# SashaYerashoff/evo-ssearch

Measured on NVIDIA B200. Metric: flat-IP top-k queries/sec @10M x 512 k=48, higher is better.
Workload: dtype f32

## Files before the change

evo-ssearch_b200/csrc/evs_api.cu:

```cuda
#include <errno.h>
#include <float.h>
#include <stdarg.h>
#include <stdio.h>
#include <stdlib.h>
#include <string.h>
#include <fcntl.h>
#include <sys/stat.h>
#include <unistd.h>

#include <atomic>
#include <mutex>
#include <new>
#include <string>
#include <thread>
#include <utility>
#include <vector>

#include "evs_internal.h"

using namespace evs;

static thread_local char t_err[512] = "";

static int fail(int code, const char* fmt, ...) {
// ... 1015 lines not shown
            const int rc2 = barrier_scan_done(idx->device, st);
            if (!rc) rc = rc2;
        }
        return rc;
    }
    const int kp = kp_override ? kp_override : pi.kp;
    const bool bf16 = idx->storage == EVS_STORE_BF16_F32;
    const bool shadow = pi.shadow && kp_override == 0;
    const bool scan_bf16 = bf16 && !shadow && kp_override == 0;
    const void* scan_rows = shadow ? (const void*)idx->xi8 : scan_bf16 ? idx->xb16 : (const void*)idx->xb32;
    const int qpp = shadow ? 1 : max_queries_per_pass(idx->d, scan_bf16);
    ScanPlan plan;
    CU(plan_scan(idx->ntotal, idx->d, shadow ? SCAN_I8 : scan_bf16, kp, qpp, idx->sm_count, tune, &plan));
    const int64_t chunk_cap = nq < kQueryChunk ? nq : kQueryChunk;
    int rc = ensure_dev(reinterpret_cast<unsigned long long**>(&idx->lists), &idx->lists_cap, (size_t)chunk_cap * plan.grid * kp);
    if (rc) return rc;
    if (kp_override == 0) {
        if ((rc = ensure_dev(&idx->margins_dev, &idx->margins_cap, (size_t)nq))) return rc;
        idx->last_nq = nq;
    }
    const bool fused = (kp_override ? (tune.fuse_finalize && nq == 1 && plan.variant == 1) : pi.fused) && !scan_only;
    if (out.x && out.x->merge_D && !fused) return fail(EVS_ECUDA, "internal: the exchange expected a fused single-query search");
    const float err_coef = (scan_bf16 || shadow) ? 0.f : gemv_err_coef(idx->d);
    if (shadow && !(fused && tune.pool_select && kp == 64))
        return fail(EVS_ECUDA, "internal: the int8 scan copy is searched by the fused pool kernel only");

    for (int64_t c0 = 0; c0 < nq; c0 += kQueryChunk) {
        const int64_t cn = (nq - c0) < kQueryChunk ? (nq - c0) : kQueryChunk;
        const float* qc = q_dev + (size_t)c0 * idx->d;
        ProfileScope prof;
        if ((rc = prof.begin(idx, profile, st))) return rc;
        FinalizeParams f = make_finalize(idx, idx->lists, plan.grid, kp, qc, k, out, c0, nq, err_coef);
        if (shadow) {
            f.shadow_emax = reinterpret_cast<const float*>(idx->words + W_EMAX);
            f.wide = idx->words + W_WIDE;
        }
        for (int64_t p0 = 0; p0 < cn; p0 += qpp) {
            ScanArgs a;
            a.xb = scan_rows;
            a.xs = shadow ? idx->xs8 : nullptr;
            a.is_bf16 = scan_bf16;
            a.is_i8 = shadow;
            a.n = idx->ntotal;
            a.d = idx->d;
            a.xq = qc;
            a.q0 = (int)p0;
            a.nq_pass = (int)((cn - p0) < qpp ? (cn - p0) : qpp);
            a.lists = idx->lists;
            a.kp = kp;
            if (fused) {
                a.fuse = &f;
                a.ticket = idx->words + W_TICKET;
                if (tune.pool_select && kp == 64) {
                    const size_t need = scan_pool_words(plan) + (shadow ? (size_t)idx->ntotal : 0);
                    if (idx->pool_cap < need) {
                        if (idx->pool) CU(cudaFree(idx->pool));
                        idx->pool = nullptr;
                        idx->pool_cap = 0;
                        CU(cudaMalloc(reinterpret_cast<void**>(&idx->pool), need * 8));
                        CU(cudaMemsetAsync(idx->pool, 0, need * 8, st));
                        idx->pool_cap = need;
                    }
                    a.pool = idx->pool;
                    if (small_shard_applies(idx, tune, kp, plan)) {
                        a.small_fast_cap = tune.small_fast_cap > 0 ? tune.small_fast_cap : 1;
                        if (out.q_host != nullptr) {
                            a.q_inline = out.q_host;
                            f.done_flag = out.done_flag;
                            f.done_seq = out.done_seq;
                        }
                    }
                }
                if (out.q_host != nullptr && a.q_inline == nullptr)
                    return fail(EVS_ECUDA, "internal: the host search expected the small-shard kernel");
                if (tune.scan_dynamic > 1 || (tune.scan_dynamic == 1 && a.pool != nullptr)) {
                    a.next_chunk = idx->words + W_NEXT_CHUNK;
                    a.chunk_groups = tune.scan_chunk_groups > 0 ? tune.scan_chunk_groups : 2;
                }
                if (tune.scan_clock) {
                    if ((rc = ensure_dev(&idx->cta_clock, &idx->cta_clock_cap, (size_t)plan.grid * 2 + 16))) return rc;
                    idx->cta_clock_n = plan.grid;
                    a.cta_clock = idx->cta_clock;
                    f.dbg = idx->cta_clock + (size_t)plan.grid * 2 + 8;
                }
            }
            CU(launch_scan(a, &plan, st));
        }
        if ((rc = prof.end(st))) return rc;
        if (scan_only || fused) continue;
        CU(launch_finalize(f, cn, st));
    }
    return EVS_OK;
}

__global__ void fill_final_kernel(float* D, long long* I, long long count) {
    for (long long i = (long long)blockIdx.x * blockDim.x + threadIdx.x; i < count; i += (long long)gridDim.x * blockDim.x) {
        D[i] = -FLT_MAX;
        I[i] = -1;
    }
}
__global__ void fill_partial_kernel(double* S, long long* I, long long count) {
    for (long long i = (long long)blockIdx.x * blockDim.x + threadIdx.x; i < count; i += (long long)gridDim.x * blockDim.x) {
        S[i] = -DBL_MAX;
        I[i] = -1;
    }
}

// ... 984 lines not shown
```

evo-ssearch_b200/csrc/evs_finalize.cuh:

```cuda
#pragma once
#include <float.h>

#include <type_traits>

#include "evs_common.cuh"
#include "evs_internal.h"

namespace evs {

__device__ __forceinline__ void st_release_sys_u64(unsigned long long* p, unsigned long long v) {
    asm volatile("st.release.sys.global.u64 [%0], %1;" ::"l"(p), "l"(v) : "memory");
}
__device__ __forceinline__ unsigned long long ld_acquire_sys_u64(const unsigned long long* p) {
    unsigned long long v;
    asm volatile("ld.acquire.sys.global.u64 %0, [%1];" : "=l"(v) : "l"(p) : "memory");
    return v;
}

__device__ __forceinline__ u64 score_rank_key(double s) { return f64_to_ordered(s == 0.0 ? 0.0 : s); }
__device__ __forceinline__ int better_i(u64 oa, long long ia, u64 ob, long long ib) {
    return (int)(oa > ob) | ((int)(oa == ob) & (int)(ia < ib));
}
__device__ __forceinline__ double widen_f32(float f) {
    const uint32_t u = __float_as_uint(f);
// ... 165 lines not shown
            }
            __nanosleep(20);
        }
        const double sv = __longlong_as_double((long long)(((unsigned long long)a.z << 32) | a.x));
        const long long iv = (long long)(((unsigned long long)b.z << 32) | b.x);
        sc[e] = sv;
        id[e] = iv;
        ok[e] = iv >= 0 ? score_rank_key(sv) : 0ull;
    }
    __syncthreads();
    if (*fail) {
        for (int r = threadIdx.x; r < k; r += blockDim.x) {
            D[(size_t)qi * k + r] = -FLT_MAX;
            I[(size_t)qi * k + r] = -1;
        }
        if (threadIdx.x == 0 && x.status) {
            *reinterpret_cast<volatile int*>(x.status) = *fail;
            __threadfence_system();
        }
        return;
    }
    for (int e = threadIdx.x; e < m; e += blockDim.x) {
        if (id[e] < 0) continue;
        atomicAdd(nvalid, 1);
        const int part = e / k;
        const long long it = id[e];
        const u64 ot = ok[e];
        int rank = e - part * k;
        for (int pp = 0; pp < x.world; pp++) {
            if (pp == part) continue;
            const int base = pp * k;
            int lo = 0, hi = k;
            while (lo < hi) {
                const int mid = (lo + hi) >> 1;
                const bool beats = id[base + mid] >= 0 && better_i(ok[base + mid], id[base + mid], ot, it);
                if (beats) lo = mid + 1;
                else hi = mid;
            }
            rank += lo;
        }
        if (rank < k) {
            D[(size_t)qi * k + rank] = (float)sc[e];
            I[(size_t)qi * k + rank] = it;
        }
    }
    __syncthreads();
    for (int r = *nvalid + threadIdx.x; r < k; r += blockDim.x) {
        D[(size_t)qi * k + r] = -FLT_MAX;
        I[(size_t)qi * k + r] = -1;
    }
}

template <int MAXR = 4, int UW = 0>
__device__ __forceinline__ void finalize_rank_emit(const FinalizeParams& p, long long qi, const u64* A, FinalizeShared* sh, double* sc,
                                                   long long* id, u64* ok, const double* qs, unsigned char* scratch, int kp_use = 0,
                                                   float shadow_E = 0.f, u64 cut = 0ull) {
    const int t = threadIdx.x, nt = blockDim.x;
    const int warp = t >> 5, lane = t & 31, nwarps = nt >> 5;
    const int kp = kp_use > 0 ? kp_use : p.kp;
    const float* xb32 = reinterpret_cast<const float*>(p.xb);
    const bool fastw = p.special != nullptr && __ldg(p.special) == 0u;
    auto rescore = [&](auto rtag, auto ftag) {
        constexpr int R = decltype(rtag)::value;
        constexpr bool FAST = decltype(ftag)::value;
        for (int c = R * warp; c < kp; c += R * nwarps) {
            u64 key[R];
            long long row[R];
            const float* xr[R];
            double sv[R];
#pragma unroll
            for (int r = 0; r < R; r++) {
                key[r] = (c + r < kp) ? A[c + r] : 0ull;
                row[r] = key[r] ? (long long)key_row(key[r]) : -1;
                xr[r] = (key[r] && !p.xb_is_bf16) ? xb32 + (size_t)row[r] * p.d : nullptr;
            }
            canon32_dot_multi<R, FAST, UW>(xr, qs, p.d, lane, sv);
            if (p.xb_is_bf16) {
                const __nv_bfloat16* xb16 = reinterpret_cast<const __nv_bfloat16*>(p.xb);
#pragma unroll
                for (int r = 0; r < R; r++) sv[r] = key[r] ? canon32_dot_bf16(xb16 + (size_t)row[r] * p.d, qs, p.d, lane) : -DBL_MAX;
            }
            if (lane == 0) {
#pragma unroll
                for (int r = 0; r < R; r++)
                    if (c + r < kp) {
                        sc[c + r] = sv[r];
                        id[c + r] = row[r];
                        ok[c + r] = row[r] >= 0 ? score_rank_key(sv[r]) : 0ull;
                    }
            }
        }
    };
    if (MAXR < 4 || 2 * nwarps >= kp) {
        if (fastw) rescore(std::integral_constant<int, 2>{}, std::true_type{});
        else rescore(std::integral_constant<int, 2>{}, std::false_type{});
    } else {
        if (fastw) rescore(std::integral_constant<int, MAXR < 4 ? 2 : 4>{}, std::true_type{});
        else rescore(std::integral_constant<int, MAXR < 4 ? 2 : 4>{}, std::false_type{});
    }
    __syncthreads();
    fin_stamp(p, 3);
    const bool want_margin = p.margins != nullptr || p.guard_count != nullptr || p.pred_slot != nullptr;
    for (int c = t; c < kp; c += nt)
        if (id[c] >= 0 && want_margin) atomicMax(&sh->maxerr, score_to_ordered((float)(sc[c] - widen_f32(key_score(A[c])))));
    __syncthreads();

    for (int c = t; c < kp; c += nt) {
        if (id[c] < 0) continue;
        atomicAdd(&sh->nvalid, 1);
        const double st = sc[c];
        const long long it = id[c];
        const u64 ot = ok[c];
        int rank = 0;
        for (int j = 0; j < kp; j++) rank += better_i(ok[j], id[j], ot, it) & (int)(id[j] >= 0);
        if (rank < p.k) {
            if (p.D) {
                p.D[(size_t)qi * p.k + rank] = (float)st;
                p.I[(size_t)qi * p.k + rank] = it + p.id_base;
            } else if (p.x.world > 0) {
                exchange_store_entry(p.x, (size_t)(p.x.q_off + qi) * p.k + rank, st, it + p.id_base, exchange_flag(p.x.seq));
            } else {
                p.P_scores[(size_t)qi * p.k + rank] = st;
                p.P_ids[(size_t)qi * p.k + rank] = it + p.id_base;
            }
            if (rank == p.k - 1 && want_margin && shadow_E > 0.f) {
                if (p.margins) p.margins[qi] = cut > 1ull ? (float)(st - widen_f32(key_score(cut))) - shadow_E : INFINITY;
            } else if (rank == p.k - 1 && want_margin) {
                const float worst = key_score(A[kp - 1]);
                const float under = fmaxf(ordered_to_score(sh->maxerr), 0.f);
                const float gap = (A[kp - 1] != 0ull) ? (float)(st - widen_f32(worst)) : INFINITY;
                const float margin = gap - under;
                if (p.margins) p.margins[qi] = margin;
                if (p.err_coef > 0.f) {
                    const float mx = p.max_norm ? *p.max_norm : 1.f;
                    const float B = sqrtf((float)sh->qnorm2) * 1.000001f * mx;
                    const bool certified = p.err_trunc > 0.f ? gap > p.err_trunc * (B + fabsf(worst)) + p.err_coef * B
                                                             : margin > p.err_coef * B;
                    if (!certified) sh->uncert = 1;
                }
            }
        }
    }
    __syncthreads();
    const int nvalid = sh->nvalid;
    for (int r = nvalid + t; r < p.k; r += nt) {
        if (p.D) {
            p.D[(size_t)qi * p.k + r] = -FLT_MAX;
            p.I[(size_t)qi * p.k + r] = -1;
        } else if (p.x.world > 0) {
            exchange_store_entry(p.x, (size_t)(p.x.q_off + qi) * p.k + r, -DBL_MAX, -1, exchange_flag(p.x.seq));
        } else {
            p.P_scores[(size_t)qi * p.k + r] = -DBL_MAX;
            p.P_ids[(size_t)qi * p.k + r] = -1;
        }
    }
    if (t == 0 && p.margins && nvalid < p.k) p.margins[qi] = INFINITY;
    if (t == 0) {
        const bool over = p.overflow != nullptr && p.overflow[qi] != 0;
        if (sh->uncert || over) {
            if (p.guard_count) {
                const int slot = atomicAdd(p.guard_count, 1);
                if (slot < p.guard_cap) {
                    p.guard_slot[qi] = slot;
                    p.guard_q[slot] = (int)qi;
                } else {
                    p.guard_slot[qi] = -2;
                    if (p.guard_cap > 0 && p.uncertified) atomicAdd(p.uncertified, 1ull);
                }
            } else if (p.uncertified) {
                atomicAdd(p.uncertified, 1ull);
            }
        }
    }
    fin_stamp(p, 4);
    if (p.x.world > 0 && p.D == nullptr) {
        if (t == 0) sh->nvalid = 0;
        if (p.x.merge_D != nullptr) {
            __syncthreads();
            exchange_merge(p.x, p.x.q_off + qi, p.x.nq_total, p.k, p.x.merge_D, p.x.merge_I, scratch,
                           &sh->fail, &sh->nvalid);
        }
    }
}



__device__ __forceinline__ void finalize_query(const FinalizeParams& p, long long qi, const u64* __restrict__ lists,
                                               unsigned char* smem_raw) {
    const int t = threadIdx.x, nt = blockDim.x;
    const int warp = t >> 5, lane = t & 31, nwarps = nt >> 5;
    const int kp = p.kp, L = p.L;
    const int scap = finalize_surv_cap(L, kp);
    FinalizeShared* sh = reinterpret_cast<FinalizeShared*>(smem_raw);
    u64* surv = reinterpret_cast<u64*>(smem_raw + sizeof(FinalizeShared));
    u64* pre = surv + finalize_surv_slots(L, kp);
    int* deep = reinterpret_cast<int*>(pre + 2 * (size_t)L);
    double* sc = reinterpret_cast<double*>(pre + 2 * (size_t)L + finalize_deep_slots(L));
    long long* id = reinterpret_cast<long long*>(sc + kp);
    u64* ok = reinterpret_cast<u64*>(id + kp);
    double* qs = reinterpret_cast<double*>(ok + kp);

    for (int l = t; l < L; l += nt) {
        const ulonglong2 v = __ldcg(reinterpret_cast<const ulonglong2*>(lists + (size_t)l * kp));
        pre[2 * l] = v.x;
        pre[2 * l + 1] = v.y;
    }
    if (qi == 0 && t == 0 && p.guard_count_next) *p.guard_count_next = 0;
    __syncthreads();
    fin_stamp(p, 0);
    if (p.err_coef > 0.f && warp == 0) {
        double s2 = 0.0;
        for (int i = lane; i < p.d; i += 32) s2 = fma(qs[i], qs[i], s2);
#pragma unroll
        for (int off = 16; off >= 1; off >>= 1) s2 += __shfl_xor_sync(0xffffffffu, s2, off);
        if (lane == 0) sh->qnorm2 = s2;
    }
    int hs = 1;
    while ((L / (hs * 2)) * 10 >= kp * 23) hs <<= 1;
    for (int attempt = 0; attempt < 2; attempt++) {
        if (attempt == 1) {
            if (sh->nsurv <= scap || hs == 1) break;
            __syncthreads();
            if (t == 0) {
                sh->nsurv = 0;
                sh->ndeep = 0;
                sh->T0 = 0ull;
            }
            hs = 1;
            __syncthreads();
        }
        const int Ls = (L + hs - 1) / hs;
        if (Ls >= kp) {
            int nper = 1;
            while (nper < 32 && nper * 2 * Ls <= nt) nper <<= 1;
            const int part = t & (nper - 1);
            for (int l0 = 0; l0 < Ls; l0 += nt / nper) {
                const int l = l0 + t / nper;
// ... 93 lines not shown
```

evo-ssearch_b200/csrc/evs_scan.cuh:

```cuda
#pragma once
#include "evs_common.cuh"
#include "evs_finalize.cuh"

namespace evs {

struct ScanParams {
    const void* xb;
    const float* xs;
    long long n;
    int d;
    const float* xq;
    int q0;
    u64* lists;
    int lists_stride_q;
    int kp;
    int tile_rows;
    int stages;
    unsigned* ticket;
    unsigned* next_chunk;
    int chunk_groups;
    const int* qmap;
    const int* nactive;
    int qcap;
    unsigned long long* cta_clock;
// ... 325 lines not shown
                if (threadIdx.x == 0) {
                    *p.ticket = 0u;
                    if (p.next_chunk) *p.next_chunk = 0u;
                }
                __threadfence();
                if (p.cta_clock && threadIdx.x == 0) {
                    unsigned long long* x = p.cta_clock + 2 * gridDim.x;
                    x[0] = globaltimer_ns();
                    x[2] = t_fin;
                    x[3] = t_merged;
                    x[4] = p.cta_clock[2 * blockIdx.x + 1];
                }
                finalize_prologue(f, p.q0, smem_raw);
                __syncthreads();
                finalize_query(f, p.q0, f.lists + (size_t)p.q0 * f.L * f.kp, smem_raw);
                if (p.cta_clock && threadIdx.x == 0) p.cta_clock[2 * gridDim.x + 1] = globaltimer_ns();
            }
        }
    }
}

constexpr int POOL_SLOTS = 64;
constexpr int POOL_GSTRIDE = 16;
constexpr int POOL_COUNT = POOL_SLOTS * POOL_GSTRIDE;
constexpr int POOL_TICKET = POOL_COUNT + 16;
constexpr int POOL_HDR = POOL_TICKET + 16;
constexpr int POOL_SURV = 2048;
constexpr int POOL_KPMAX = 256;
__host__ __device__ inline size_t pool_finalize_smem_bytes(int kp, int d, int world_k) {
    size_t surv = (size_t)(POOL_SURV + kp) * 8;
    const size_t merge = (size_t)world_k * 24 + 8;
    if (merge > surv) surv = (merge + 7) & ~(size_t)7;
    return sizeof(FinalizeShared) + surv + (3 * (size_t)kp + (size_t)d) * 8 + 16;
}

__host__ __device__ inline size_t small_query_smem_offset(int kp, int d, int world_k) {
    return (pool_finalize_smem_bytes(kp, d, world_k) + 15) & ~(size_t)15;
}

__device__ __forceinline__ float shadow_bound_i8(const FinalizeParams& f, double dq2, double qh2) {
    const double dq = sqrt(dq2) * (1.0 + 0x1p-20), qh = sqrt(qh2) * (1.0 + 0x1p-20);
    const double nx = (double)__ldg(f.max_norm) * (1.0 + 0x1p-7);
    const double em = (double)__ldg(f.shadow_emax);
    const double e = (dq * nx + qh * em + 0x1p-22 * qh * (nx + em)) * (1.0 + 0x1p-20) + 0x1p-117;
    return __double2float_ru(e);
}
__device__ __forceinline__ u64 key_lowered(u64 t, float twoE) {
    if (twoE == 0.f || t == 0ull) return t;
    if (!(twoE <= FLT_MAX)) return 1ull;
    const uint32_t o = score_to_ordered(__fsub_rd(key_score(t), twoE));
    return o == 0u ? 1ull : ((u64)o << 32);
}

__device__ __forceinline__ int pool_wide_rounds(const FinalizeParams& f, const u64* S, unsigned m, u64 cut, u64* cand, u64* keep,
                                             double* sc, long long* id, u64* ok, const double* qs, int* s_n) {
    const int t = threadIdx.x, nt = blockDim.x, warp = t >> 5, lane = t & 31, nwarps = nt >> 5;
    const float* xb32 = reinterpret_cast<const float*>(f.xb);
    const bool fastw = f.special != nullptr && __ldg(f.special) == 0u;
    const int lines = (f.d * 4 + 127) / 128;
    int fill = 0;
    u64 key = (t < 128 && t < m) ? __ldcg(S + t) : 0ull;
    for (unsigned b0 = 0; b0 < m; b0 += 128) {
        const u64 nkey = (t < 128 && b0 + 128 + t < m) ? __ldcg(S + b0 + 128 + t) : 0ull;
        const bool mem = key != 0ull && key >= cut;
        if (mem) {
            const char* row = reinterpret_cast<const char*>(f.xb) + (size_t)key_row(key) * f.d * 4;
            for (int i = 0; i < lines; i++) asm volatile("prefetch.global.L2 [%0];" ::"l"(row + (size_t)i * 128));
        }
        const int nb = __syncthreads_count(mem);
        if (fill + nb > POOL_KPMAX) {
            for (int c = 2 * warp; c < fill; c += 2 * nwarps) {
                long long row[2];
                const float* xr[2];
                double sv[2];
#pragma unroll
                for (int r = 0; r < 2; r++) {
                    row[r] = c + r < fill ? (long long)key_row(cand[c + r]) : -1;
                    xr[r] = row[r] >= 0 ? xb32 + (size_t)row[r] * f.d : nullptr;
                }
                if (fastw) canon32_dot_multi<2, true>(xr, qs, f.d, lane, sv);
                else canon32_dot_multi<2, false>(xr, qs, f.d, lane, sv);
                if (lane == 0)
#pragma unroll
                    for (int r = 0; r < 2; r++)
                        if (c + r < fill) {
                            sc[c + r] = sv[r];
                            id[c + r] = row[r];
                            ok[c + r] = score_rank_key(sv[r]);
                        }
            }
            __syncthreads();
            for (int c = t; c < fill; c += nt) {
                int rank = 0;
                for (int j = 0; j < fill; j++) rank += better_i(ok[j], id[j], ok[c], id[c]);
                if (rank < f.k) keep[rank] = cand[c];
            }
            __syncthreads();
            fill = fill < f.k ? fill : f.k;
            for (int c = t; c < fill; c += nt) cand[c] = keep[c];
        }
        if (t == 0) *s_n = fill;
        __syncthreads();
        if (mem) cand[atomicAdd(s_n, 1)] = key;
        fill += nb;
        key = nkey;
        __syncthreads();
    }
    return fill;
}

__device__ __forceinline__ u64 warp_min_u64(u64 v) {
#pragma unroll
    for (int off = 16; off >= 1; off >>= 1) {
        const u64 o = __shfl_xor_sync(0xffffffffu, v, off);
        v = o < v ? o : v;
    }
    return v;
}
__device__ __forceinline__ u64 pool_tau(const u64* G, int lane, u64& ga, u64& gb) {
    ga = __ldcg(G + (size_t)lane * POOL_GSTRIDE);
    gb = __ldcg(G + (size_t)(lane + 32) * POOL_GSTRIDE);
    return warp_min_u64(ga < gb ? ga : gb);
}
__device__ __forceinline__ void pool_publish(u64* G, u64 key, u64 ga, u64 gb) {
    const int slot = (int)((~(uint32_t)key) & (POOL_SLOTS - 1));
    const u64 va = __shfl_sync(0xffffffffu, ga, slot & 31), vb = __shfl_sync(0xffffffffu, gb, slot & 31);
    const u64 cur = slot < 32 ? va : vb;
    if (key != 0ull && key > cur) atomicMax(reinterpret_cast<unsigned long long*>(G + (size_t)slot * POOL_GSTRIDE), (unsigned long long)key);
}

template <typename T, int NV>
__global__ void __launch_bounds__(256, ScanOcc<T, 1, NV>::value) scan_pool_kernel(ScanParams p, FinalizeParams f, u64* pool) {
    extern __shared__ __align__(128) unsigned char smem_raw[];
    __shared__ int s_last, s_ns, s_wcnt[9];
    __shared__ unsigned s_base;
    __shared__ u64 s_tau, s_wtau[8];
    __shared__ float s_twoE;
    constexpr bool I8 = sizeof(T) == 1;
    constexpr int QREGS = NV * Elem<T>::VEC;
    constexpr int RPG_RAW = (100 - QREGS) / (NV * 4);
    constexpr int RPG = I8 ? I8Lane<NV>::ROWS : (RPG_RAW < 1 ? 1 : (RPG_RAW > 4 ? 4 : RPG_RAW));
    constexpr int KP = 64, CAPW = 128;
    const int warp = threadIdx.x >> 5, lane = threadIdx.x & 31;
    const int nwarps = blockDim.x >> 5;
    u64* G = pool;
    unsigned* count = reinterpret_cast<unsigned*>(pool + POOL_COUNT);
    unsigned* ticket = reinterpret_cast<unsigned*>(pool + POOL_TICKET);
    u64* S = pool + POOL_HDR;
    u64* buf = reinterpret_cast<u64*>(smem_raw) + (size_t)warp * CAPW;

    asm volatile("griddepcontrol.wait;" ::: "memory");
    asm volatile("griddepcontrol.launch_dependents;" ::: "memory");
    unsigned long long t_start = 0, t_loop = 0, t_app = 0;
    if (p.cta_clock && threadIdx.x == 0) t_start = globaltimer_ns();

    const long long total_warps = (long long)gridDim.x * nwarps;
    const long long gw = (long long)blockIdx.x * nwarps + warp;
    const long long ngroups = (p.n + RPG - 1) / RPG;
    QueryRegs<T, 1, NV> q;
    q.load(p.xq, p.q0, p.d, lane);
    int cnt = 0;
    bool early = false;
    if (lane == 0) s_wtau[warp] = 0ull;
    double* qs;
    {
        size_t surv_bytes = (size_t)(POOL_SURV + KP) * 8;
        const size_t merge = (size_t)f.x.world * f.k * 24 + 8;
        if (merge > surv_bytes) surv_bytes = (merge + 7) & ~(size_t)7;
        qs = reinterpret_cast<double*>(smem_raw + sizeof(FinalizeShared) + surv_bytes + 3 * (size_t)POOL_KPMAX * 8);
        const float* qf = p.xq + (size_t)p.q0 * p.d;
        for (int i = threadIdx.x; i < p.d; i += blockDim.x) qs[i] = (double)qf[i];
    }
    bool bounded = false;
    if constexpr (I8) {
        if (f.shadow_emax != nullptr) {
            bounded = true;
            __syncthreads();
            double dq2 = 0.0, qh2 = 0.0;
            for (int i = lane; i < p.d; i += 32) {
                const double qh = (double)q.sq * (double)i8_query_code((float)qs[i], q.sq);
                dq2 = fma(qs[i] - qh, qs[i] - qh, dq2);
                qh2 = fma(qh, qh, qh2);
            }
#pragma unroll
            for (int off = 16; off >= 1; off >>= 1) {
                dq2 += __shfl_xor_sync(0xffffffffu, dq2, off);
                qh2 += __shfl_xor_sync(0xffffffffu, qh2, off);
            }
            if (lane == 0) s_twoE = 2.f * shadow_bound_i8(f, dq2, qh2);
        }
    }
    if (!bounded && threadIdx.x == 0) s_twoE = 0.f;
    u64 tcut = 0ull;

    auto compact = [&]() {
        __syncwarp();
        for (int i = cnt + lane; i < CAPW; i += 32) buf[i] = 0ull;
        warp_bitonic_sort_desc(buf, CAPW, lane);
        u64 ga, gb;
        const u64 tg = pool_tau(G, lane, ga, gb);
        pool_publish(G, lane < 8 ? buf[lane] : 0ull, ga, gb);
        const u64 tau = umax64(s_wtau[warp], umax64(buf[KP - 1], tg));
        __syncwarp();
        if (lane == 0) s_wtau[warp] = tau;
        tcut = key_lowered(tau, f.shadow_emax ? s_twoE : 0.f);
        cnt = 0;
#pragma unroll
        for (int h = 0; h < CAPW / 32; h++) {
            const u64 kh = buf[lane + 32 * h];
            cnt += __popc(__ballot_sync(0xffffffffu, kh != 0ull && kh >= tcut));
        }
        if (cnt > CAPW - 32) {
            unsigned b = 0;
            if (lane == 0) b = atomicAdd(count, (unsigned)(cnt - KP));
            b = __shfl_sync(0xffffffffu, b, 0);
            for (int i = KP + lane; i < cnt; i += 32) S[b + i - KP] = buf[i];
            cnt = KP;
            __syncwarp();
        }
    };

    auto publish_first16 = [&]() {
        early = true;
        __syncwarp();
        u64 mx = lane < 16 ? buf[lane] : 0ull;
#pragma unroll
        for (int off = 8; off >= 1; off >>= 1) mx = umax64(mx, __shfl_xor_sync(0xffffffffu, mx, off));
        if (lane == 0) atomicMax(reinterpret_cast<unsigned long long*>(G + (size_t)((~(uint32_t)mx) & (POOL_SLOTS - 1)) * POOL_GSTRIDE), (unsigned long long)mx);
    };
    const long long dyn_groups = (p.next_chunk && ngroups >= 32 * total_warps) ? (ngroups / 8 > 64 * total_warps ? 64 * total_warps : ngroups / 8) : 0;
    const long long static_end = ngroups - dyn_groups;
    long long next = -1;
    if (dyn_groups > 0 && lane == 0) next = (long long)atomicAdd(p.next_chunk, 1u);
    if constexpr (I8) {
        typedef I8Lane<NV> L;
        constexpr int R = L::ROWS, RSH = L::RSH;
        const int8_t* codes = reinterpret_cast<const int8_t*>(p.xb);
        const int rl = lane >> RSH;
        const bool rep = (lane & ((1 << RSH) - 1)) == 0;
        struct Group {
            unsigned w[R][L::WORDS];
            float sr;
        };
        auto load = [&](Group& b, long long g) {
            const long long r0 = g * R;
            b.sr = __ldg(p.xs + (r0 + rl < p.n ? r0 + rl : p.n - 1));
#pragma unroll
            for (int r = 0; r < R; r++) {
                const long long row = r0 + r < p.n ? r0 + r : p.n - 1;
                L::load(codes + (size_t)row * p.d, lane, b.w[r]);
            }
        };
        auto score = [&](const Group& b, long long g) {
            constexpr int M = NV <= 2 ? R : 2 * R;
            int v[M];
#pragma unroll
            for (int r = 0; r < R; r++) {
                int ih = 0, il = 0;
#pragma unroll
                for (int w = 0; w < L::WORDS; w++) {
                    ih = __dp4a((int)b.w[r][w], q.h[w], ih);
                    il = __dp4a((int)b.w[r][w], q.l[w], il);
                }
                if constexpr (NV <= 2) v[r] = ih * 256 + il;
                else {
                    v[2 * r] = ih;
                    v[2 * r + 1] = il;
                }
            }
// ... 61 lines not shown
#pragma unroll
                for (int j = 0; j < NV; j++) {
                    if constexpr (sizeof(T) == 4) raw[r][j] = ldg_stream_f4(src + 32 * j);
                    else raw[r][j] = ldg_stream_u4(src + 32 * j);
                }
            }
#pragma unroll
            for (int r = 0; r < RPG; r++) {
                float s[1];
                row_scores<T, 1, NV>(raw[r], q, s);
                if (r0 + r < p.n) {
                    const u64 key = make_key(s[0], (uint32_t)(r0 + r));
                    if (key > tcut) {
                        if (lane == 0) buf[cnt] = key;
                        if (++cnt == CAPW) compact();
                        else if (cnt == 16 && !early) publish_first16();
                    }
                }
            }
        };
        for (long long g = gw; g < static_end; g += total_warps) do_group(g);
        if (dyn_groups > 0) {
            const long long C = p.chunk_groups;
            const long long nchunks = (dyn_groups + C - 1) / C;
            long long chunk = __shfl_sync(0xffffffffu, next, 0);
            while (chunk < nchunks) {
                if (lane == 0) next = (long long)atomicAdd(p.next_chunk, 1u);
                const long long g0 = static_end + chunk * C;
                const long long gend = g0 + C < ngroups ? g0 + C : ngroups;
                for (long long g = g0; g < gend; g++) do_group(g);
                chunk = __shfl_sync(0xffffffffu, next, 0);
            }
        }
    }
    if (p.cta_clock && threadIdx.x == 0) t_loop = globaltimer_ns();

    {
        __syncwarp();
        u64 ga, gb;
        const u64 tg = pool_tau(G, lane, ga, gb);
        tcut = key_lowered(umax64(s_wtau[warp], tg), f.shadow_emax ? s_twoE : 0.f);
        int kept = 0;
        for (int i0 = 0; i0 < cnt; i0 += 32) {
            const u64 key = (i0 + lane < cnt) ? buf[i0 + lane] : 0ull;
            const bool keep = key != 0ull && key >= tcut;
            const unsigned m = __ballot_sync(0xffffffffu, keep);
            __syncwarp();
            if (keep) buf[kept + __popc(m & ((1u << lane) - 1u))] = key;
            pool_publish(G, keep ? key : 0ull, ga, gb);
            kept += __popc(m);
            __syncwarp();
        }
        if (lane == 0) s_wcnt[warp] = kept;
    }
    if (p.cta_clock && threadIdx.x == 0) {
        t_app = globaltimer_ns();
        p.cta_clock[2 * blockIdx.x] = t_start;
        p.cta_clock[2 * blockIdx.x + 1] = t_loop;
    }
    __syncthreads();
    if (threadIdx.x == 0) {
        int total = 0;
        for (int w = 0; w < nwarps; w++) {
            const int c = s_wcnt[w];
            s_wcnt[w] = total;
            total += c;
        }
        s_wcnt[nwarps] = total;
        s_base = total ? atomicAdd(count, (unsigned)total) : 0u;
    }
    __syncthreads();
    {
        const int off = s_wcnt[warp], end = warp + 1 < nwarps ? s_wcnt[warp + 1] : s_wcnt[nwarps];
        for (int i = lane; i < end - off; i += 32) S[s_base + off + i] = buf[i];
    }

    __threadfence();
    __syncthreads();
    if (threadIdx.x == 0) s_last = atomicAdd(ticket, 1u) == gridDim.x - 1 ? 1 : 0;
    __syncthreads();
    if (!s_last) return;

    __threadfence();
    const int t = threadIdx.x, nt = blockDim.x;
    FinalizeShared* sh = reinterpret_cast<FinalizeShared*>(smem_raw);
    u64* surv = reinterpret_cast<u64*>(smem_raw + sizeof(FinalizeShared));
    size_t surv_bytes = (size_t)(POOL_SURV + KP) * 8;
    {
        const size_t merge = (size_t)f.x.world * f.k * 24 + 8;
        if (merge > surv_bytes) surv_bytes = (merge + 7) & ~(size_t)7;
    }
    double* sc = reinterpret_cast<double*>(smem_raw + sizeof(FinalizeShared) + surv_bytes);
    long long* id = reinterpret_cast<long long*>(sc + POOL_KPMAX);
    u64* ok = reinterpret_cast<u64*>(id + POOL_KPMAX);
    if (p.cta_clock && t == 0) {
        unsigned long long* x = p.cta_clock + 2 * gridDim.x;
        x[0] = globaltimer_ns();
        x[2] = t_app;
        x[3] = t_app;
        x[4] = t_loop;
    }
    const unsigned m = __ldcg(count);
    u64 spec[POOL_SURV / 2 / 256];
#pragma unroll
    for (int u = 0; u < POOL_SURV / 2 / 256; u++) spec[u] = __ldcg(S + t + 256 * u);
    if (warp == 0) {
        u64 ga, gb;
        const u64 tg = pool_tau(G, lane, ga, gb);
        if (lane == 0) s_tau = tg;
    }
    if (t == 0) {
        s_ns = 0;
        sh->nsurv = 0;
        sh->nvalid = 0;
        sh->maxerr = 0u;
        sh->ndeep = 0;
        sh->T0 = 0ull;
        sh->qnorm2 = 0.0;
        sh->fail = 0;
        sh->uncert = 0;
    }
    __syncthreads();
    if (f.err_coef > 0.f && warp == 0) {
        double s2 = 0.0;
        for (int i = lane; i < f.d; i += 32) s2 = fma(qs[i], qs[i], s2);
#pragma unroll
        for (int off = 16; off >= 1; off >>= 1) s2 += __shfl_xor_sync(0xffffffffu, s2, off);
        if (lane == 0) sh->qnorm2 = s2;
// ... 74 lines not shown
            }
            if (t == 0) s_ns = 0;
            __syncthreads();
            if (t < 2 * KP) {
                const u64 mine = cmax[t];
                int r = 0;
                for (int j = 0; j < 2 * KP; j++) r += cmax[j] > mine ? 1 : 0;
                if (r == KP - 1) s_tau = mine;
            }
            __syncthreads();
            const u64 T = s_tau;
            u64* dst = surv + POOL_SURV / 2;
            for (int i = t; i < ns; i += nt) {
                const u64 key = surv[i];
                if (key >= T) dst[atomicAdd(&s_ns, 1)] = key;
            }
            __syncthreads();
            src = dst;
            nsrc = s_ns;
        }
        if (!f.xb_is_bf16 && nsrc <= 4 * KP) {
            const int lines = (f.d * 4 + 127) / 128;
            for (int i = t; i < nsrc * lines; i += nt) {
                const char* row = reinterpret_cast<const char*>(f.xb) + (size_t)key_row(src[i / lines]) * f.d * 4 + (size_t)(i % lines) * 128;
                asm volatile("prefetch.global.L2 [%0];" ::"l"(row));
            }
        }
        u64* top = surv + POOL_SURV;
        for (int i = t; i < KP; i += nt) top[i] = 0ull;
        __syncthreads();
        for (int i = t; i < nsrc; i += nt) {
            const u64 key = src[i];
            int r = 0;
            for (int j = 0; j < nsrc; j++) r += src[j] > key ? 1 : 0;
            if (r < KP) top[r] = key;
        }
        __syncthreads();
        A = top;
    } else {
        for (int i = ns + t; i < POOL_SURV; i += nt) surv[i] = 0ull;
        for (int size = 2; size <= POOL_SURV; size <<= 1)
            for (int stride = size >> 1; stride > 0; stride >>= 1) {
                __syncthreads();
                for (int e = t; e < (POOL_SURV >> 1); e += nt) {
                    const int i = bitonic_low(e, stride);
                    cmpx_desc(surv, i, i + stride, (i & size) == 0);
                }
            }
        __syncthreads();
        A = surv;
    }
    fin_stamp(f, 2);
    const float twoE = s_twoE;
    if (f.shadow_emax == nullptr) {
        finalize_rank_emit<(ScanOcc<T, 1, NV>::value >= 4 ? 2 : 4)>(f, p.q0, A, sh, sc, id, ok, qs, reinterpret_cast<unsigned char*>(surv));
    } else {
        const u64 kth = A[f.k - 1];
        __syncthreads();
        const u64 cut = kth ? key_lowered(kth, twoE) : 1ull;
        u64* cand = surv;
        if (t == 0) s_ns = 0;
        __syncthreads();
        for (unsigned i = t; i < m; i += nt) {
            const u64 key = __ldcg(S + i);
            if (key != 0ull && key >= cut) {
                const int pos = atomicAdd(&s_ns, 1);
                if (pos < POOL_KPMAX) cand[pos] = key;
            }
        }
        __syncthreads();
        int nc = s_ns;
        if (t == 0 && f.wide) {
            f.wide[1] = (unsigned)nc;
            if (nc > POOL_KPMAX) atomicAdd(f.wide, 1u);
        }
        if (nc > POOL_KPMAX) nc = pool_wide_rounds(f, S, m, cut, cand, surv + POOL_KPMAX, sc, id, ok, qs, &s_ns);
        const int lines = (f.d * 4 + 127) / 128;
        for (int i = t; i < nc * lines; i += nt) {
            const char* row = reinterpret_cast<const char*>(f.xb) + (size_t)key_row(cand[i / lines]) * f.d * 4 + (size_t)(i % lines) * 128;
            asm volatile("prefetch.global.L2 [%0];" ::"l"(row));
        }
        for (int i = nc + t; i < KP; i += nt) cand[i] = 0ull;
        __syncthreads();
        finalize_rank_emit<(ScanOcc<T, 1, NV>::value >= 4 ? 2 : 4)>(f, p.q0, cand, sh, sc, id, ok, qs, reinterpret_cast<unsigned char*>(surv),
                                                                     nc > KP ? nc : KP, twoE * 0.5f, cut);
    }
    if (p.cta_clock && t == 0) p.cta_clock[2 * gridDim.x + 1] = globaltimer_ns();
}

__device__ __forceinline__ const u64* pool_rank_survivors(const FinalizeParams& f, u64* surv, int ns, int* s_ns, u64* s_tau, u64* cmax) {
    constexpr int KP = 64;
    const int t = threadIdx.x, nt = blockDim.x;
    if (ns <= POOL_SURV / 2) {
        const u64* src = surv;
        int nsrc = ns;
        if (ns > 3 * KP) {
            if (t < 2 * KP) {
                u64 mx = 0ull;
                for (int i = t; i < ns; i += 2 * KP) mx = umax64(mx, surv[i]);
                cmax[t] = mx;
            }
            if (t == 0) *s_ns = 0;
            __syncthreads();
            if (t < 2 * KP) {
                const u64 mine = cmax[t];
                int r = 0;
                for (int j = 0; j < 2 * KP; j++) r += cmax[j] > mine ? 1 : 0;
                if (r == KP - 1) *s_tau = mine;
            }
            __syncthreads();
            const u64 T = *s_tau;
            u64* dst = surv + POOL_SURV / 2;
            for (int i = t; i < ns; i += nt) {
                const u64 key = surv[i];
                if (key >= T) dst[atomicAdd(s_ns, 1)] = key;
            }
            __syncthreads();
            src = dst;
            nsrc = *s_ns;
        }
        if (!f.xb_is_bf16 && nsrc <= 4 * KP) {
            const int lines = (f.d * 4 + 127) / 128;
            for (int i = t; i < nsrc * lines; i += nt) {
                const char* row = reinterpret_cast<const char*>(f.xb) + (size_t)key_row(src[i / lines]) * f.d * 4 + (size_t)(i % lines) * 128;
                asm volatile("prefetch.global.L2 [%0];" ::"l"(row));
            }
        }
        u64* top = surv + POOL_SURV;
        for (int i = t; i < KP; i += nt) top[i] = 0ull;
        __syncthreads();
        for (int i = t; i < nsrc; i += nt) {
            const u64 key = src[i];
            int r = 0;
            for (int j = 0; j < nsrc; j++) r += src[j] > key ? 1 : 0;
            if (r < KP) top[r] = key;
        }
        __syncthreads();
        return top;
// ... 356 lines not shown
```

Before: 1223.

## Score shadow survivors exactly in scan CTAs and finalize via streaming window

In the int8-shadow bounded path, each scan CTA now computes exact fp32 dot products for the candidates it appends to the pool and stores them in a parallel score array (the pool allocation is doubled to hold it). Spilled candidates are marked as unscored. The last-CTA finalize streams survivors above the cut into a bounded window, rescores only the unscored ones, and periodically reduces the window to the top-k. This replaces the serial candidate gather plus full rescoring in finalize. The rescore work is spread across all CTAs and overlaps with the scan, at the cost of extra memory, exact scoring of candidates that may later be pruned, and more complex synchronisation.

```diff
diff --git a/evo-ssearch_b200/csrc/evs_api.cu b/evo-ssearch_b200/csrc/evs_api.cu
--- a/evo-ssearch_b200/csrc/evs_api.cu
+++ b/evo-ssearch_b200/csrc/evs_api.cu
@@ -1091,7 +1091,7 @@
                 a.fuse = &f;
                 a.ticket = idx->words + W_TICKET;
                 if (tune.pool_select && kp == 64) {
-                    const size_t need = scan_pool_words(plan) + (shadow ? (size_t)idx->ntotal : 0);
+                    const size_t need = scan_pool_words(plan) + (shadow ? 2 * (size_t)idx->ntotal : 0);
                     if (idx->pool_cap < need) {
                         if (idx->pool) CU(cudaFree(idx->pool));
                         idx->pool = nullptr;
diff --git a/evo-ssearch_b200/csrc/evs_finalize.cuh b/evo-ssearch_b200/csrc/evs_finalize.cuh
--- a/evo-ssearch_b200/csrc/evs_finalize.cuh
+++ b/evo-ssearch_b200/csrc/evs_finalize.cuh
@@ -241,12 +241,10 @@
 }
 
 template <int MAXR = 4, int UW = 0>
-__device__ __forceinline__ void finalize_rank_emit(const FinalizeParams& p, long long qi, const u64* A, FinalizeShared* sh, double* sc,
-                                                   long long* id, u64* ok, const double* qs, unsigned char* scratch, int kp_use = 0,
-                                                   float shadow_E = 0.f, u64 cut = 0ull) {
+__device__ __forceinline__ void finalize_rescore(const FinalizeParams& p, const u64* A, int kp, FinalizeShared* sh, double* sc,
+                                                 long long* id, u64* ok, const double* qs) {
     const int t = threadIdx.x, nt = blockDim.x;
     const int warp = t >> 5, lane = t & 31, nwarps = nt >> 5;
-    const int kp = kp_use > 0 ? kp_use : p.kp;
     const float* xb32 = reinterpret_cast<const float*>(p.xb);
     const bool fastw = p.special != nullptr && __ldg(p.special) == 0u;
     auto rescore = [&](auto rtag, auto ftag) {
@@ -289,11 +287,19 @@
     }
     __syncthreads();
     fin_stamp(p, 3);
+}
+
+template <bool SCAN_KEYS = true>
+__device__ __forceinline__ void finalize_emit(const FinalizeParams& p, long long qi, const u64* A, int kp, FinalizeShared* sh,
+                                              const double* sc, const long long* id, const u64* ok, unsigned char* scratch,
+                                              float shadow_E = 0.f, u64 cut = 0ull) {
+    const int t = threadIdx.x, nt = blockDim.x;
     const bool want_margin = p.margins != nullptr || p.guard_count != nullptr || p.pred_slot != nullptr;
-    for (int c = t; c < kp; c += nt)
-        if (id[c] >= 0 && want_margin) atomicMax(&sh->maxerr, score_to_ordered((float)(sc[c] - widen_f32(key_score(A[c])))));
-    __syncthreads();
-
+    if constexpr (SCAN_KEYS) {
+        for (int c = t; c < kp; c += nt)
+            if (id[c] >= 0 && want_margin) atomicMax(&sh->maxerr, score_to_ordered((float)(sc[c] - widen_f32(key_score(A[c])))));
+        __syncthreads();
+    }
     for (int c = t; c < kp; c += nt) {
         if (id[c] < 0) continue;
         atomicAdd(&sh->nvalid, 1);
@@ -372,6 +378,15 @@
     }
 }
 
+template <int MAXR = 4, int UW = 0>
+__device__ __forceinline__ void finalize_rank_emit(const FinalizeParams& p, long long qi, const u64* A, FinalizeShared* sh, double* sc,
+                                                   long long* id, u64* ok, const double* qs, unsigned char* scratch, int kp_use = 0,
+                                                   float shadow_E = 0.f, u64 cut = 0ull) {
+    const int kp = kp_use > 0 ? kp_use : p.kp;
+    finalize_rescore<MAXR, UW>(p, A, kp, sh, sc, id, ok, qs);
+    finalize_emit(p, qi, A, kp, sh, sc, id, ok, scratch, shadow_E, cut);
+}
+
 
 
 __device__ __forceinline__ void finalize_query(const FinalizeParams& p, long long qi, const u64* __restrict__ lists,
diff --git a/evo-ssearch_b200/csrc/evs_scan.cuh b/evo-ssearch_b200/csrc/evs_scan.cuh
--- a/evo-ssearch_b200/csrc/evs_scan.cuh
+++ b/evo-ssearch_b200/csrc/evs_scan.cuh
@@ -401,61 +401,113 @@
     return o == 0u ? 1ull : ((u64)o << 32);
 }
 
-__device__ __forceinline__ int pool_wide_rounds(const FinalizeParams& f, const u64* S, unsigned m, u64 cut, u64* cand, u64* keep,
-                                             double* sc, long long* id, u64* ok, const double* qs, int* s_n) {
-    const int t = threadIdx.x, nt = blockDim.x, warp = t >> 5, lane = t & 31, nwarps = nt >> 5;
-    const float* xb32 = reinterpret_cast<const float*>(f.xb);
-    const bool fastw = f.special != nullptr && __ldg(f.special) == 0u;
-    const int lines = (f.d * 4 + 127) / 128;
-    int fill = 0;
-    u64 key = (t < 128 && t < m) ? __ldcg(S + t) : 0ull;
-    for (unsigned b0 = 0; b0 < m; b0 += 128) {
-        const u64 nkey = (t < 128 && b0 + 128 + t < m) ? __ldcg(S + b0 + 128 + t) : 0ull;
-        const bool mem = key != 0ull && key >= cut;
-        if (mem) {
-            const char* row = reinterpret_cast<const char*>(f.xb) + (size_t)key_row(key) * f.d * 4;
-            for (int i = 0; i < lines; i++) asm volatile("prefetch.global.L2 [%0];" ::"l"(row + (size_t)i * 128));
-        }
-        const int nb = __syncthreads_count(mem);
-        if (fill + nb > POOL_KPMAX) {
-            for (int c = 2 * warp; c < fill; c += 2 * nwarps) {
-                long long row[2];
-                const float* xr[2];
+__device__ __forceinline__ void pool_score_rows(const FinalizeParams& f, long long row0, long long row1, const double* qs, int lane,
+                                                double (&sv)[2]) {
+    const float* xb = reinterpret_cast<const float*>(f.xb);
+    const float* xr[2] = {xb + (size_t)row0 * f.d, row1 >= 0 ? xb + (size_t)row1 * f.d : nullptr};
+    if (f.special != nullptr && __ldg(f.special) == 0u) canon32_dot_multi<2, true>(xr, qs, f.d, lane, sv);
+    else canon32_dot_multi<2, false>(xr, qs, f.d, lane, sv);
+}
+constexpr long long POOL_UNSCORED = 0x7FF4D15C0DE5C0DEll;
+
+constexpr int POOL_WCAP = 640;
+constexpr int POOL_WPER = 8;
+__device__ __forceinline__ int pool_exact_window(const FinalizeParams& f, const u64* S, const double* X, unsigned m, u64 cut,
+                                                 const double* qs, double* wsc, long long* wid, u64* wok, double* ksc, long long* kid, u64* kok,
+                                                 int* s_n, int* s_c, int* s_u) {
+    const int t = threadIdx.x, nt = blockDim.x, lane = t & 31;
+    if (t == 0) {
+        *s_n = 0;
+        *s_c = 0;
+        *s_u = 0;
+    }
+    __syncthreads();
+    const unsigned batch = (unsigned)nt * POOL_WPER;
+    u64 key[POOL_WPER];
+    double xs[POOL_WPER];
+#pragma unroll
+    for (int u = 0; u < POOL_WPER; u++) {
+        const unsigned i = t + nt * u;
+        key[u] = i < m ? __ldcg(S + i) : 0ull;
+        xs[u] = i < m ? __ldcg(X + i) : 0.0;
+    }
+    for (unsigned b0 = 0; b0 < m; b0 += batch) {
+        unsigned pend = 0u;
+#pragma unroll
+        for (int u = 0; u < POOL_WPER; u++) {
+            const bool mem = key[u] != 0ull && key[u] >= cut;
+            pend |= mem ? 1u << u : 0u;
+        }
+        if (pend) atomicAdd(s_c, __popc(pend));
+#pragma unroll
+        for (int u = 0; u < POOL_WPER; u++) {
+            unsigned need = __ballot_sync(0xffffffffu, ((pend >> u) & 1u) && __double_as_longlong(xs[u]) == POOL_UNSCORED);
+            if (need != 0u && lane == 0) atomicAdd(s_u, __popc(need));
+            while (need) {
+                const int l0 = __ffs(need) - 1;
+                need &= need - 1u;
+                const int l1 = need ? __ffs(need) - 1 : -1;
+                if (need) need &= need - 1u;
+                const u64 k0 = __shfl_sync(0xffffffffu, key[u], l0), k1 = __shfl_sync(0xffffffffu, key[u], l1 < 0 ? l0 : l1);
                 double sv[2];
-#pragma unroll
-                for (int r = 0; r < 2; r++) {
-                    row[r] = c + r < fill ? (long long)key_row(cand[c + r]) : -1;
-                    xr[r] = row[r] >= 0 ? xb32 + (size_t)row[r] * f.d : nullptr;
-                }
-                if (fastw) canon32_dot_multi<2, true>(xr, qs, f.d, lane, sv);
-                else canon32_dot_multi<2, false>(xr, qs, f.d, lane, sv);
-                if (lane == 0)
-#pragma unroll
-                    for (int r = 0; r < 2; r++)
-                        if (c + r < fill) {
-                            sc[c + r] = sv[r];
-                            id[c + r] = row[r];
-                            ok[c + r] = score_rank_key(sv[r]);
-                        }
-            }
-            __syncthreads();
-            for (int c = t; c < fill; c += nt) {
+                pool_score_rows(f, (long long)key_row(k0), l1 < 0 ? -1 : (long long)key_row(k1), qs, lane, sv);
+                if (lane == l0) xs[u] = sv[0];
+                if (lane == l1) xs[u] = sv[1];
+            }
+        }
+        u64 nkey[POOL_WPER];
+        double nxs[POOL_WPER];
+#pragma unroll
+        for (int u = 0; u < POOL_WPER; u++) {
+            const unsigned i = b0 + batch + t + nt * u;
+            nkey[u] = i < m ? __ldcg(S + i) : 0ull;
+            nxs[u] = i < m ? __ldcg(X + i) : 0.0;
+        }
+        for (;;) {
+#pragma unroll
+            for (int u = 0; u < POOL_WPER; u++) {
+                const bool want = (pend >> u) & 1u;
+                const unsigned bal = __ballot_sync(0xffffffffu, want);
+                if (bal == 0u) continue;
+                int base = 0;
+                if (lane == 0) base = atomicAdd(s_n, __popc(bal));
+                base = __shfl_sync(0xffffffffu, base, 0);
+                const int pos = base + __popc(bal & ((1u << lane) - 1u));
+                if (want && pos < POOL_WCAP) {
+                    wsc[pos] = xs[u];
+                    wid[pos] = (long long)key_row(key[u]);
+                    wok[pos] = score_rank_key(xs[u]);
+                    pend &= ~(1u << u);
+                }
+            }
+            if (!__syncthreads_or(pend != 0u)) break;
+            const int n = POOL_WCAP;
+            for (int c = t; c < n; c += nt) {
                 int rank = 0;
-                for (int j = 0; j < fill; j++) rank += better_i(ok[j], id[j], ok[c], id[c]);
-                if (rank < f.k) keep[rank] = cand[c];
-            }
-            __syncthreads();
-            fill = fill < f.k ? fill : f.k;
-            for (int c = t; c < fill; c += nt) cand[c] = keep[c];
-        }
-        if (t == 0) *s_n = fill;
-        __syncthreads();
-        if (mem) cand[atomicAdd(s_n, 1)] = key;
-        fill += nb;
-        key = nkey;
-        __syncthreads();
-    }
-    return fill;
+                for (int j = 0; j < n; j++) rank += better_i(wok[j], wid[j], wok[c], wid[c]);
+                if (rank < f.k) {
+                    ksc[rank] = wsc[c];
+                    kid[rank] = wid[c];
+                    kok[rank] = wok[c];
+                }
+            }
+            __syncthreads();
+            for (int c = t; c < f.k; c += nt) {
+                wsc[c] = ksc[c];
+                wid[c] = kid[c];
+                wok[c] = kok[c];
+            }
+            if (t == 0) *s_n = f.k;
+            __syncthreads();
+        }
+#pragma unroll
+        for (int u = 0; u < POOL_WPER; u++) {
+            key[u] = nkey[u];
+            xs[u] = nxs[u];
+        }
+    }
+    const int n = *s_n;
+    return n < POOL_WCAP ? n : POOL_WCAP;
 }
 
 __device__ __forceinline__ u64 warp_min_u64(u64 v) {
@@ -481,7 +533,7 @@
 template <typename T, int NV>
 __global__ void __launch_bounds__(256, ScanOcc<T, 1, NV>::value) scan_pool_kernel(ScanParams p, FinalizeParams f, u64* pool) {
     extern __shared__ __align__(128) unsigned char smem_raw[];
-    __shared__ int s_last, s_ns, s_wcnt[9];
+    __shared__ int s_last, s_ns, s_nc, s_nu, s_wcnt[9];
     __shared__ unsigned s_base;
     __shared__ u64 s_tau, s_wtau[8];
     __shared__ float s_twoE;
@@ -541,6 +593,7 @@
     }
     if (!bounded && threadIdx.x == 0) s_twoE = 0.f;
     u64 tcut = 0ull;
+    auto pool_x = [&]() { return reinterpret_cast<double*>(pool + POOL_HDR + (size_t)gridDim.x * (blockDim.x >> 5) * CAPW + p.n); };
 
     auto compact = [&]() {
         __syncwarp();
@@ -564,6 +617,10 @@
             if (lane == 0) b = atomicAdd(count, (unsigned)(cnt - KP));
             b = __shfl_sync(0xffffffffu, b, 0);
             for (int i = KP + lane; i < cnt; i += 32) S[b + i - KP] = buf[i];
+            if constexpr (I8) {
+                double* X = pool_x() + b - KP;
+                for (int i = KP + lane; i < cnt; i += 32) X[i] = __longlong_as_double(POOL_UNSCORED);
+            }
             cnt = KP;
             __syncwarp();
         }
@@ -731,6 +788,14 @@
             __syncwarp();
         }
         if (lane == 0) s_wcnt[warp] = kept;
+        if constexpr (I8)
+            if (bounded) {
+                const int lines = (p.d * 4 + 127) / 128;
+                for (int i = lane; i < kept * lines; i += 32) {
+                    const char* row = reinterpret_cast<const char*>(f.xb) + (size_t)key_row(buf[i / lines]) * p.d * 4 + (size_t)(i % lines) * 128;
+                    asm volatile("prefetch.global.L2 [%0];" ::"l"(row));
+                }
+            }
     }
     if (p.cta_clock && threadIdx.x == 0) {
         t_app = globaltimer_ns();
@@ -753,6 +818,25 @@
         const int off = s_wcnt[warp], end = warp + 1 < nwarps ? s_wcnt[warp + 1] : s_wcnt[nwarps];
         for (int i = lane; i < end - off; i += 32) S[s_base + off + i] = buf[i];
     }
+    if constexpr (I8)
+        if (bounded) {
+            const int total = s_wcnt[nwarps];
+            const u64* bufs = reinterpret_cast<const u64*>(smem_raw);
+            double* X = pool_x() + s_base;
+            auto key_at = [&](int j) {
+                int w = 0;
+                for (int v = 1; v < nwarps; v++) w = s_wcnt[v] <= j ? v : w;
+                return bufs[(size_t)w * CAPW + j - s_wcnt[w]];
+            };
+            for (int j = 2 * warp; j < total; j += 2 * nwarps) {
+                double sv[2];
+                pool_score_rows(f, (long long)key_row(key_at(j)), j + 1 < total ? (long long)key_row(key_at(j + 1)) : -1, qs, lane, sv);
+                if (lane == 0) {
+                    X[j] = sv[0];
+                    if (j + 1 < total) X[j + 1] = sv[1];
+                }
+            }
+        }
 
     __threadfence();
     __syncthreads();
@@ -933,38 +1017,29 @@
     }
     fin_stamp(f, 2);
     const float twoE = s_twoE;
-    if (f.shadow_emax == nullptr) {
+    if (!bounded) {
         finalize_rank_emit<(ScanOcc<T, 1, NV>::value >= 4 ? 2 : 4)>(f, p.q0, A, sh, sc, id, ok, qs, reinterpret_cast<unsigned char*>(surv));
     } else {
         const u64 kth = A[f.k - 1];
         __syncthreads();
         const u64 cut = kth ? key_lowered(kth, twoE) : 1ull;
-        u64* cand = surv;
-        if (t == 0) s_ns = 0;
-        __syncthreads();
-        for (unsigned i = t; i < m; i += nt) {
-            const u64 key = __ldcg(S + i);
-            if (key != 0ull && key >= cut) {
-                const int pos = atomicAdd(&s_ns, 1);
-                if (pos < POOL_KPMAX) cand[pos] = key;
-            }
-        }
-        __syncthreads();
-        int nc = s_ns;
-        if (t == 0 && f.wide) {
-            f.wide[1] = (unsigned)nc;
-            if (nc > POOL_KPMAX) atomicAdd(f.wide, 1u);
-        }
-        if (nc > POOL_KPMAX) nc = pool_wide_rounds(f, S, m, cut, cand, surv + POOL_KPMAX, sc, id, ok, qs, &s_ns);
-        const int lines = (f.d * 4 + 127) / 128;
-        for (int i = t; i < nc * lines; i += nt) {
-            const char* row = reinterpret_cast<const char*>(f.xb) + (size_t)key_row(cand[i / lines]) * f.d * 4 + (size_t)(i % lines) * 128;
-            asm volatile("prefetch.global.L2 [%0];" ::"l"(row));
-        }
-        for (int i = nc + t; i < KP; i += nt) cand[i] = 0ull;
-        __syncthreads();
-        finalize_rank_emit<(ScanOcc<T, 1, NV>::value >= 4 ? 2 : 4)>(f, p.q0, cand, sh, sc, id, ok, qs, reinterpret_cast<unsigned char*>(surv),
-                                                                     nc > KP ? nc : KP, twoE * 0.5f, cut);
+        double* wsc = reinterpret_cast<double*>(surv);
+        long long* wid = reinterpret_cast<long long*>(wsc + POOL_WCAP);
+        u64* wok = reinterpret_cast<u64*>(wid + POOL_WCAP);
+        const int nw = pool_exact_window(f, S, pool_x(), m, cut, qs, wsc, wid, wok, sc, id, ok, &s_ns, &s_nc, &s_nu);
+        if (t == 0) {
+            const unsigned nc = (unsigned)s_nc;
+            if (f.wide) {
+                f.wide[1] = nc;
+                if (nc > POOL_KPMAX) atomicAdd(f.wide, 1u);
+            }
+            if (f.dbg) {
+                f.dbg[5] = m;
+                f.dbg[6] = (unsigned)s_nu;
+            }
+        }
+        fin_stamp(f, 3);
+        finalize_emit<false>(f, p.q0, nullptr, nw, sh, wsc, wid, wok, reinterpret_cast<unsigned char*>(surv), twoE * 0.5f, cut);
     }
     if (p.cta_clock && t == 0) p.cta_clock[2 * gridDim.x + 1] = globaltimer_ns();
 }
```

New measurement: 1283, median of 6. +4.9%, better.
